# timmh/biolith

Hardware: AMD Instinct MI355X
Metric: effective samples/sec (psi) for occu NUTS, 10k sites x 5 visits (higher is better)
Workload: dtype f32; 1 GPU; biolith simulate(n_sites=10000, n_site_covs=3, n_obs_covs=3, 5 visits, seed 0); fit(occu): NUTS 4 chains per GPU x (1000 warmup + 1000 draws), one step = one full fit; chains_per_gpu=4, total_chains=4, num_warmup=1000, num_samples=1000, parallelism=chains x1 (1 process per GPU), wgs_per_chain=27, gather=none (one rank), env_overrides=

## Files before the change

biolith_amd/_ffi.py:

```python
from __future__ import annotations

import ctypes as C
import os
import threading

_HERE = os.path.dirname(os.path.abspath(__file__))
LIB_PATH = os.environ.get("BIOLITH_HIP_LIB") or os.path.join(_HERE, "lib", "libbiolith_hip.so")

BL_OK, BL_ERR_INVALID, BL_ERR_NO_DEVICE, BL_ERR_UNSUPPORTED, BL_ERR_TIMEOUT, BL_ERR_ABORTED, BL_ERR_BUSY, BL_ERR_COMM = range(8)
COMM_ID_BYTES = 128
RNG_STREAMS_PER_CHAIN = 64
MAX_COVS = 16
PSIS_MAX_DRAWS = 8192
SUMMARY_MAX_RANKS = 16
RICHNESS_MAX_SPECIES = 32


class EngineError(RuntimeError):

    def __init__(self, code: int, message: str):
        super().__init__(f"biolith_hip error {code}: {message}")
        self.code = code


# ... 35 lines not shown
        ("inv_mass", C.POINTER(C.c_float)), ("n_leapfrog", C.POINTER(C.c_int64)),
    ]


EXPORTS = (
    "bl_abi_version", "bl_last_error", "bl_device_count", "bl_dataset_create", "bl_dataset_create_rn", "bl_dataset_create_dyn", "bl_dataset_destroy",
    "bl_dataset_param_dim", "bl_logp_grad", "bl_nuts_run", "bl_nuts_launch", "bl_nuts_poll",
    "bl_nuts_abort", "bl_nuts_wait", "bl_nuts_fetch", "bl_nuts_elapsed_ms", "bl_nuts_device_draws",
    "bl_nuts_geometry", "bl_nuts_lane_group", "bl_nuts_kernel_name", "bl_nuts_debug_counters", "bl_deterministic", "bl_predict", "bl_predict_counts", "bl_predict_scores", "bl_dataset_create_fp", "bl_dataset_create_cop", "bl_dataset_create_nmix", "bl_dataset_create_re", "bl_dataset_create_re_fp", "bl_dataset_create_nmix_re", "bl_dataset_create_rn_re", "bl_dataset_create_rn_fp", "bl_dataset_create_cop_re", "bl_dataset_create_cs", "bl_dataset_create_comb", "bl_dataset_set_prior_family", "bl_rng_streams", "bl_adaptation_schedule",
    "bl_comm_rccl_version", "bl_comm_unique_id", "bl_comm_init_rank", "bl_comm_init_all", "bl_comm_info", "bl_comm_destroy",
    "bl_gather_draws", "bl_result_block_layout", "bl_gather_unpack", "bl_host_alloc", "bl_host_free",
    "bl_nuts_env_overrides", "bl_env_overrides", "bl_site_posterior", "bl_abundance_posterior", "bl_path_posterior",
    "bl_score_posterior", "bl_count_posterior", "bl_predict_comb", "bl_deterministic_comb", "bl_predictive_check",
    "bl_predictive_density", "bl_psis_loo", "bl_predictive_check_counts", "bl_site_summary", "bl_regional_totals",
    "bl_site_diagnostics", "bl_response_curves", "bl_trajectory_totals", "bl_species_richness",
    "bl_residual_moran",
)

_lib = None
_lock = threading.Lock()


def load():
    global _lib
    with _lock:
        if _lib is not None:
            return _lib
        if not os.path.exists(LIB_PATH):
            raise RuntimeError(
                f"{LIB_PATH} is missing: build the HIP engine with `make -C biolith_amd/csrc -j8` "
                "(or `python -c 'import __graft_entry__ as g; g.build()'`). "
# ... 39 lines not shown
        L.bl_logp_grad.argtypes = [vp, C.c_int, dp, dp, dp, C.c_int]
        L.bl_nuts_run.argtypes = [vp, C.POINTER(bl_nuts_config), C.POINTER(bl_nuts_output)]
        L.bl_nuts_launch.argtypes = [vp, C.POINTER(bl_nuts_config), vp]
        L.bl_nuts_poll.argtypes = [vp, ip]
        L.bl_nuts_abort.argtypes = [vp]
        L.bl_nuts_wait.argtypes = [vp]
        L.bl_nuts_fetch.argtypes = [vp, C.POINTER(bl_nuts_output)]
        L.bl_nuts_elapsed_ms.argtypes = [vp, fp]
        L.bl_nuts_device_draws.argtypes = [vp, C.POINTER(vp), C.POINTER(C.c_size_t)]
        L.bl_nuts_geometry.argtypes = [vp, ip, ip, ip, ip, ip]
        L.bl_nuts_lane_group.argtypes = [vp, ip, ip]
        L.bl_nuts_kernel_name.argtypes = [vp, C.c_char_p, C.c_int]
        if hasattr(L, "bl_nuts_env_overrides"):
            L.bl_nuts_env_overrides.argtypes = [vp, C.c_char_p, C.c_int]
            L.bl_env_overrides.argtypes = [C.c_char_p, C.c_int]
        L.bl_nuts_debug_counters.argtypes = [vp, C.POINTER(C.c_int64), C.c_int]
        L.bl_host_alloc.argtypes = [C.c_size_t, C.POINTER(C.c_void_p)]
        L.bl_host_free.argtypes = [C.c_void_p]
        L.bl_deterministic.argtypes = [vp, C.c_int, fp, fp, fp]
        L.bl_predict.argtypes = [vp, C.c_int, fp, C.c_uint64, C.POINTER(C.c_uint8), C.POINTER(C.c_uint8)]
        L.bl_predict_counts.argtypes = [vp, C.c_int, fp, C.c_uint64, C.POINTER(C.c_int32), C.POINTER(C.c_int32)]
        L.bl_predict_scores.argtypes = [vp, C.c_int, fp, C.c_uint64, C.POINTER(C.c_uint8), C.POINTER(C.c_uint8), fp]
        L.bl_predict_comb.argtypes = [vp, C.c_int, fp, C.c_uint64, C.POINTER(C.c_uint8), C.POINTER(C.c_uint8), C.POINTER(C.c_uint8), fp]
        L.bl_deterministic_comb.argtypes = [vp, C.c_int, fp, fp, fp, fp]
        L.bl_predictive_check.argtypes = [vp, C.c_int, fp, C.c_uint64, C.POINTER(C.c_uint8), dp, dp]
        L.bl_predictive_check_counts.argtypes = [vp, C.c_int, fp, C.c_uint64, C.POINTER(C.c_int32), dp, dp]
        L.bl_predictive_density.argtypes = [vp, C.c_int, fp, C.c_uint64, C.POINTER(C.c_uint8), C.c_int, dp, dp, dp]
        L.bl_site_summary.argtypes = [vp, C.c_int, fp, C.c_int, C.POINTER(C.c_int32), dp, dp, fp, dp, dp, fp]
        L.bl_site_diagnostics.argtypes = [vp, C.c_int, fp, C.c_int, dp, dp, dp, dp, dp, dp, dp, dp]
        L.bl_regional_totals.argtypes = [vp, C.c_int, fp, C.c_uint64, C.c_int, C.POINTER(C.c_int32), dp, dp, dp]
# ... 9 lines not shown
        L.bl_score_posterior.argtypes = [vp, C.c_int, fp, C.c_uint64, fp, fp, C.POINTER(C.c_uint8), fp, C.POINTER(C.c_uint8)]
        L.bl_count_posterior.argtypes = [vp, C.c_int, fp, C.c_uint64, fp, fp, C.POINTER(C.c_uint8), fp, C.POINTER(C.c_int32)]
        L.bl_rng_streams.argtypes = [C.c_uint64, C.c_int, C.c_int, C.POINTER(C.c_uint32)]
        L.bl_adaptation_schedule.argtypes = [C.c_int, C.POINTER(C.c_int32), C.POINTER(C.c_int32), C.c_int]
        u8p = C.POINTER(C.c_uint8)
        L.bl_comm_rccl_version.argtypes = [ip]
        L.bl_comm_unique_id.argtypes = [u8p]
        L.bl_comm_init_rank.argtypes = [u8p, C.c_int, C.c_int, C.c_int, C.POINTER(vp)]
        L.bl_comm_init_all.argtypes = [C.c_int, ip, C.POINTER(vp)]
        L.bl_comm_info.argtypes = [vp, ip, ip, ip, dp]
        L.bl_comm_destroy.argtypes = [vp]
        L.bl_gather_draws.argtypes = [C.POINTER(vp), C.POINTER(vp), C.c_int, C.POINTER(C.c_int32), C.POINTER(bl_nuts_output)]
        L.bl_result_block_layout.argtypes = [C.c_int, C.c_int, C.c_int, C.POINTER(C.c_uint64)]
        L.bl_gather_unpack.argtypes = [C.c_void_p, C.c_uint64, C.c_int, C.POINTER(C.c_int32), C.c_int, C.c_int, C.POINTER(bl_nuts_output)]
        for name in EXPORTS:
            if name != "bl_last_error" and (hasattr(L, name) or name not in ("bl_nuts_env_overrides", "bl_env_overrides")):
                getattr(L, name).restype = C.c_int
        if L.bl_abi_version() != 1:
            raise RuntimeError("libbiolith_hip.so ABI version mismatch")
        _lib = L
        return _lib


def check(rc: int):
    if rc != BL_OK:
        msg = load().bl_last_error().decode("utf-8", "replace")
        if rc == BL_ERR_INVALID:
            raise ValueError(f"biolith_hip: {msg}")
        if rc == BL_ERR_UNSUPPORTED:
            raise NotImplementedError(f"biolith_hip: {msg}")
        if rc in (BL_ERR_TIMEOUT,):
# ... 9 lines not shown
```

biolith_amd/csrc/biolith_hip.hip:

```cpp
#include "../../include/biolith_hip.h"

#include <hip/hip_runtime.h>

#include <algorithm>
#include <climits>
#include <cmath>
#include <cstdarg>
#include <cstdio>
#include <cstdlib>
#include <cstring>
#include <string>
#include <vector>

#include "logp_kernel.hpp"
#include "re_kernel.hpp"
#include "nuts_kernel.hpp"
#include "predict.hpp"
#include "site_posterior.hpp"
#include "abundance_posterior.hpp"
#include "path_posterior.hpp"
#include "score_posterior.hpp"
#include "count_posterior.hpp"
#include "comb_predict.hpp"
#include "predictive_check.hpp"
// ... 1895 lines not shown
                 o_cold = carve(sizeof(BlNutsCold));
    if (off > ds->run_bytes) {
        if (ds->d_run) hipFree(ds->d_run);
        ds->d_run = nullptr; ds->run_bytes = 0;
        BL_HIP(hipMalloc(&ds->d_run, off));
        ds->run_bytes = off;
    }
    char *base = (char *)ds->d_run;
    ds->d_draws = (float *)(base + o_draws); ds->d_div = (unsigned char *)(base + o_div); ds->d_steps = (int *)(base + o_steps);
    ds->d_acc = (float *)(base + o_acc); ds->d_pot = (float *)(base + o_pot); ds->d_eps = (float *)(base + o_eps);
    ds->d_minv = (float *)(base + o_minv); ds->d_nleap = (long long *)(base + o_nleap); ds->d_status = (int *)(base + o_status);
    ds->d_rng = (uint32_t *)(base + o_rng); ds->d_init = (float *)(base + o_init); ds->d_dbg = (long long *)(base + o_dbg); ds->d_loc = (int *)(base + o_loc);
    int pitch = nvp;
    { const char *e = bl_env(BL_ENV_PITCH); if (e && atoi(e) >= nvp && atoi(e) <= 4096) pitch = atoi(e); }
    pitch += pitch & 1;
    const size_t xb = align256((size_t)C * BL_XCHG_SLOTS * k * pitch * 8);
    if (xb > ds->xchg_bytes) {
        if (ds->d_xchg) hipFree(ds->d_xchg);
        ds->d_xchg = nullptr; ds->xchg_bytes = 0;
        BL_HIP(hipMalloc((void **)&ds->d_xchg, xb));
        ds->xchg_bytes = xb;
    }

    hipStream_t st = (hipStream_t)stream;
    std::vector<uint32_t> rs((size_t)C * BL_RNG_STREAMS_PER_CHAIN * 4);
    for (int c = 0; c < C; c++)
        rng_streams(cfg->seed, cfg->chain_offset + c, BL_RNG_STREAMS_PER_CHAIN, rs.data() + (size_t)c * BL_RNG_STREAMS_PER_CHAIN * 4);
    BL_HIP(hipMemcpyAsync(ds->d_rng, rs.data(), rs.size() * 4, hipMemcpyHostToDevice, st));
    if (cfg->init_theta) {
        std::vector<float> it32((size_t)C * D);
        for (size_t i = 0; i < it32.size(); i++) it32[i] = (float)cfg->init_theta[i];
// ... 218 lines not shown
{
    if (!ds) return bl_fail(BL_ERR_INVALID, "NULL argument");
    if (!ds->have_run) return bl_fail(BL_ERR_INVALID, "no NUTS launch on this handle");
    if (wgs_per_chain) *wgs_per_chain = ds->k;
    if (threads_per_wg) *threads_per_wg = ds->model == 6 ? BL_RE_NT : 64 * (ds->ncw + 1);
    if (lds_bytes) *lds_bytes = ds->lds_bytes;
    if (lds_staged) *lds_staged = ds->staged;
    if (chains_on_l2_local_exchange) {
        *chains_on_l2_local_exchange = 0;
        if (!ds->in_flight && ds->d_loc) {
            std::vector<int> loc(ds->C, 0);
            BL_HIP(hipMemcpy(loc.data(), ds->d_loc, (size_t)ds->C * 4, hipMemcpyDeviceToHost));
            for (int v : loc) *chains_on_l2_local_exchange += v;
        }
    }
    return BL_OK;
}

extern "C" int bl_deterministic(bl_dataset *ds, int n_draws, const float *draws, float *psi, float *prob_detection)
{
    if (!ds || !draws || n_draws <= 0) return bl_fail(BL_ERR_INVALID, "bl_deterministic: bad argument");
    if (ds->nsp > 1) return bl_fail(BL_ERR_UNSUPPORTED, "bl_deterministic: a joint-species handle samples; take the sites from one handle per species");
    if (ds->model == 8) return bl_fail(BL_ERR_UNSUPPORTED, "bl_deterministic: the dynamic occupancy model's sites (psi, gamma, eps) are formed by the caller from the draws");
    if (ds->model == 6 && ds->re.kind == 8)
        return bl_fail(BL_ERR_UNSUPPORTED, "bl_deterministic: occu_comb's sites (psi, PC / ARU detection probabilities) are formed by the caller from the draws");
    if (ds->in_flight) return bl_fail(BL_ERR_BUSY, "a NUTS launch is in flight on this handle");
    int rc = set_device(ds);
    if (rc || (prob_detection && (rc = upload_once(&ds->d_wraw, ds->h_wraw)))) return rc;
    BlPredictParams p = predict_params(ds, 0);
    const size_t cells = (size_t)p.T * p.N * 4;
// ... 394 lines not shown
```

biolith_amd/csrc/nuts_kernel.hpp:

```cpp
#pragma once
#include "occu_device.hpp"

#ifdef BL_STAMPS
#define BL_STAMP_DECL long long st_acc[8] = {0, 0, 0, 0, 0, 0, 0, 0}; long long st_prev = (long long)clock64(); long long st_rt0 = (long long)wall_clock64(); long long st_spins = 0; \
    long long st_kn[3] = {0, 0, 0}, st_kc[3] = {0, 0, 0}; int st_kind = 0; long long st_sub[6] = {0, 0, 0, 0, 0, 0}; long long st_t = 0; \
    long long st_ae[8] = {0, 0, 0, 0, 0, 0, 0, 0}; int st_ae_cls = -1; \
    long long st_pr[4] = {0, 0, 0, 0}; long long st_bo = 0, st_r0 = 0; bool st_first = true;
#define BL_STAMP_ROUND0 st_r0 = (long long)clock64();
#define BL_STAMP_ROUND1 { const long long st_now = (long long)clock64(); st_sub[3] += st_now - st_r0; \
    if (st_first) { st_pr[0] += st_now - st_r0; st_pr[1] += st_now - st_bo; st_pr[3]++; st_first = false; } else st_pr[2] += st_now - st_r0; }
#define BL_STAMP(i) { const long long st_now = (long long)clock64(); st_acc[i] += st_now - st_prev; \
    if (st_ae_cls >= 0 && (i) <= 1) { st_ae[st_ae_cls * 4 + 1 + ((i) & 1)] += st_now - st_prev; if ((i) == 0) st_ae[st_ae_cls * 4]++; } \
    if ((i) == 5) st_ae_cls = -1; \
    if ((i) == 1) { st_bo = st_now; st_first = true; } \
    st_prev = st_now; }
#define BL_STAMP_AFTER_END(ek) st_ae_cls = ((ek) & 16) ? 1 : (((ek) & 2) ? 0 : -1);
#define BL_STAMP_KIND(k) st_kind = (k);
#define BL_STAMP_CRIT { const long long st_now = (long long)clock64(); st_kn[st_kind]++; st_kc[st_kind] += st_now - st_prev; }
#define BL_COUNT_SPINS(n) { st_spins += (long long)(n); if (st_ae_cls >= 0) st_ae[st_ae_cls * 4 + 3] += (long long)(n); }
#define BL_SUB0 st_t = (long long)clock64();
#define BL_SUB(i) { const long long st_n2 = (long long)clock64(); st_sub[i] += st_n2 - st_t; st_t = st_n2; }
#else
#define BL_SUB0
#define BL_SUB(i)
// ... 143 lines not shown
#define BL_RESIDENT_REC 1
#endif
#ifndef BL_RESIDENT_MAX_FLOATS
#define BL_RESIDENT_MAX_FLOATS 96
#endif
#define SMALL_D_NVP(LEAN, MODEL, KS, KO) ((LEAN) && ((MODEL) == 0 || (MODEL) == 1) && (KS) + (KO) + 2 <= 8)
#ifndef BL_POLL_PAIRS
#define BL_POLL_PAIRS 1
#endif
#ifndef BL_POLL_EARLY
#define BL_POLL_EARLY 0
#endif
#ifndef BL_POLL_REFILL
#define BL_POLL_REFILL 1
#endif
__host__ __device__ __forceinline__ constexpr int bl_pair_pos(int v) { return v < 8 ? 2 * v : 2 * (v - 8) + 1; }
__host__ __device__ __forceinline__ constexpr int bl_pair_lane(int v) { return v < 8 ? v : 24 + v; }
typedef unsigned BlU4 __attribute__((ext_vector_type(4)));
#ifndef BL_OUT_DIRECT
#define BL_OUT_DIRECT 1
#endif
#ifndef BL_ABORT_DEFER
#define BL_ABORT_DEFER 0
#endif
#define BL_ABORT_LAG 8u
typedef __attribute__((address_space(1))) unsigned BlGlobalU;
typedef __attribute__((address_space(1))) unsigned char BlGlobalB;
typedef __attribute__((address_space(1))) const int BlGlobalCI;
#ifndef BL_GRP_FORM
#define BL_GRP_FORM 2
// ... 71 lines not shown
    float pend_dE = 0.f, pend_z = 0.f, pend_g = 0.f;
    double pend_U = 0.0;
    int pend_snprop = 0;
    bool init_pending = true;
    float mom_r0 = 0.f;
    double mom_kin = 0.0;
    int end_kind = 0;
    bool local = false;
    float prior_loc = 0.f, prior_isc2 = 0.f, prior_l1 = 0.f;
    double prior_const = 0.0;
    int S = 0, W = 0, total = 0, nwin = 0, win_end_cur = 0;
    float target_accept = 0.8f;

    const int nvp = SMALL_D_NVP(LEAN, MODEL, KS, KO) ? 16 : p.nvp, G = 64 / nvp;
    const int c_idx = lane & (nvp - 1), sub = lane / nvp;
    const unsigned rec_bytes = (unsigned)(p.k * p.pitch * 8);
    const unsigned char *xbase = reinterpret_cast<const unsigned char *>(p.xchg) + (size_t)chain * BL_XCHG_SLOTS * rec_bytes;
    unsigned poff[8];
    float pval[8];
#pragma unroll
    for (int q = 0; q < 8; q++) {
        const int w = q * G + sub;
        poff[q] = (unsigned)(((w < p.k ? w : p.k - 1) * p.pitch + c_idx) * 8);
        pval[q] = (w < p.k) ? 1.0f : 0.0f;
    }
    const int nq = (p.k + G - 1) / G;
    const bool one_batch = LEAN || p.k <= 8 * G;
    constexpr bool PAIRS = BL_POLL_PAIRS && SMALL_D_NVP(LEAN, MODEL, KS, KO) && multi_wg;
    unsigned ppoff[4] = {0u, 0u, 0u, 0u};
#define BL_XL(v) (PAIRS ? bl_pair_lane(v) : (v))
    if constexpr (PAIRS) {
        const int psub = (lane >> 3) & 3;
#pragma unroll
        for (int q = 0; q < 4; q++) {
            const int w = 4 * (2 * q + (lane >> 5)) + psub;
            ppoff[q] = (unsigned)(((w < p.k ? w : p.k - 1) * p.pitch + 2 * (lane & 7)) * 8);
        }
#pragma unroll
        for (int q = 0; q < 8; q++) pval[q] = (4 * q + psub < p.k) ? 1.0f : 0.0f;
    }

    if (wave == 0) {
        S = cold->num_samples; W = cold->num_warmup; total = W + S;
        target_accept = cold->target_accept; nwin = cold->nwin; win_end_cur = cold->win_end[0];
        prior_loc = beta_lane ? cold->loc_b : cold->loc_a;
        prior_isc2 = act ? (beta_lane ? cold->isc2_b : cold->isc2_a) : 0.0f;
// ... 127 lines not shown
        }
        if (pend_end) {
            const float wt = t_wt;
            float pr = fminf(1.0f, bl_exp(swt - wt));
            if (pend_sturn || pend_sdiv) pr = 0.0f;
            const float u = bl_rng_uniform(rng_u);
            if (u < pr) { t_zp = szp; t_gp = sgp; t_Up = sUp; }
            t_wt = bl_logaddexp(wt, swt);
            t_sumacc += ssumacc;
            t_nprop += pend_snprop;
        }
    };

    unsigned epoch = 0;
    bool have_pending = false, p_timed_out = false;
    double p_acc = 0.0;
    float p_cg = 0.f, p_pe2 = 0.f;
    float cz_spec = 0.f;
    int flag = 0;
    BL_STAMP_DECL
    constexpr bool SPEC = LDS && MODEL != 1;
#ifndef BL_RN_HYBRID
#define BL_RN_HYBRID 2
#endif
    constexpr bool HYBRID = BL_RN_HYBRID && LDS && MODEL == 1;
    constexpr bool POLL_FORMS = SPEC && multi_wg && KS <= 4 && KO <= 4 && MODEL != 8;
    constexpr bool POLL_EARLY = BL_POLL_EARLY && POLL_FORMS;
    constexpr bool POLL_REFILL = BL_POLL_REFILL && POLL_FORMS;
    auto poll_issue_pairs = [&](BlU4 (&v)[4], unsigned ep) {
        const int nqp = (nq + 1) >> 1;
        const __amdgpu_buffer_rsrc_t rsrc = __builtin_amdgcn_make_buffer_rsrc(const_cast<unsigned char *>(xbase), (short)0, (int)(BL_XCHG_SLOTS * rec_bytes), 0x00020000);
        const int soff = __builtin_amdgcn_readfirstlane((int)((ep & (BL_XCHG_SLOTS - 1u)) * rec_bytes));
        asm volatile("" ::: "memory");
#pragma unroll
        for (int q = 0; q < 4; q++) {
            if (q < nqp) v[q] = __builtin_amdgcn_raw_buffer_load_b128(rsrc, (int)ppoff[q], soff, 16);
            else v[q] = BlU4{0u, ep, 0u, ep};
        }
    };
    auto poll_issue_one = [&](unsigned long long (&v)[8], unsigned ep) {
        const unsigned char *rb = xbase + (ep & (BL_XCHG_SLOTS - 1u)) * rec_bytes;
#pragma unroll
        for (int q = 0; q < 8; q += 2) {
            if (q < nq) {
                v[q] = bl_poll_load(rb, poff[q]);
                v[q + 1] = bl_poll_load(rb, poff[q + 1]);
            } else {
                v[q] = (unsigned long long)ep << 32;
                v[q + 1] = (unsigned long long)ep << 32;
            }
        }
    };
    auto poll_fill_one = [&](unsigned long long (&v)[8]) {
#pragma unroll
        for (int q = 2; q < 8; q += 2)
            if (!(q < nq)) { v[q] = v[0]; v[q + 1] = v[0]; }
    };
    auto decide = [&]() {
        have_pending = false;
        const double acc = p_acc;
        const float cg = p_cg, pe2 = p_pe2;
        const double ll_tot = bl_readlane_d(acc, BL_XL(D));
        const bool abort_req = bl_readlane_d(acc, BL_XL(D + 1)) != 0.0;
        flag = 0;
        if (p_timed_out) flag = 4;
        else if (abort_req) flag = 5;
        bool new_transition = false;
        BL_STAMP_KIND(0)
        if (flag == 0) {
            if (init_pending) {
                BL_STAMP_KIND(2)
                BL_SUB0
                const double Un = -ll_tot + (double)(0.5f * bl_wave_sum(pe2)) + prior_const;
                init_pending = false;
                new_transition = true;
                t_zp = cz; t_gp = cg; t_Up = Un;
                end_kind = 1;
            } else {
// ... 100 lines not shown
                epsdir = going_right ? eps : -eps;
                snprop = 0; sturn = false; sdiv = false;
                bl_next_leaf(th, r0, gr, epsdir, minv, rh, cz);
                BL_SUB(2)
            }
        }
        if (flag != 0) end_deferred();
        if (flag != 0 && member == 0) {
            if (flag > 1 && lane == 0) atomicMax(cold->status, flag);
            if (act) cold->inv_mass[chain * D + lane] = minv;
            if (lane == 0) {
                cold->step_size[chain] = eps;
                cold->nleap[chain * 2 + 0] = ss->nleap_w;
                cold->nleap[chain * 2 + 1] = ss->nleap_s;
                cold->xcd_local[chain] = local ? 1 : 0;
            }
        }
    };

    if (wave > 0) {
        if constexpr (BL_COMPUTE_PRIO > 0 && MODEL != 1 && multi_wg) __builtin_amdgcn_s_setprio(BL_COMPUTE_PRIO);
        unsigned epoch_c = 0;
        const int lane_grp = MODEL == 1 ? bl_rn_npos(p.rn_off) : p.lane_grp;
        BlPairRec<KS, KO, (RESIDENT ? JSEL : 1)> rrec;
        bool rvalid = false;
        float rvmask = 0.0f;
        if constexpr (RESIDENT) bl_load_resident_rec(tid - 64, ld, cnt, rrec, rvalid, rvmask);
        int ab_raw = 0;
        const unsigned ab_mask = (__builtin_amdgcn_readfirstlane(wave) == 1 && member == 0) ? 0u : 0x80000000u;
        while (true) {
// ... 19 lines not shown
            if (lane == 0) tags[wave - 1] = epoch_c;
            unsigned stale = 0u;
#pragma unroll
            for (int w = 0; w < CW; w++) stale |= tags[w] ^ epoch_c;
            float row[CW];
#pragma unroll
            for (int w = 0; w < CW; w++) row[w] = part[w * part_rs];
            if (__builtin_amdgcn_readfirstlane(stale) == 0u) {
                float comp = row[0];
#pragma unroll
                for (int w = 1; w < CW; w++) comp += row[w];
                for (int sp = 1; sp < nsp; sp++) {
#pragma unroll
                    for (int w = 0; w < CW; w++) comp += part_all ? (float)part[w * part_rs + sp * BL_SP_PART(KS, KO)] : 0.0f;
                }
                if (lane > D) comp = 0.0f;
                if constexpr (ABORT_DEFER) {
                    if (lane == D + 1 && member == 0 && (epoch_c & 255u) == BL_ABORT_LAG + 1u)
                        comp = (*(__attribute__((address_space(3))) const volatile int *)(sh_flag + 2) != 0) ? 1.0f : 0.0f;
                } else {
                    if (lane == D + 1 && member == 0 && (epoch_c & 255u) == 0u)
                        comp = (__hip_atomic_load(cold->abort_flag, __ATOMIC_RELAXED, __HIP_MEMORY_SCOPE_SYSTEM) != 0) ? 1.0f : 0.0f;
                }
                if (epoch_c == 1u) {
                    const float xcc = (float)bl_xcc_id();
                    if (lane == D + 2) comp = xcc;
                    if (lane == D + 3) comp = xcc * xcc;
                }
                const unsigned char *rbase = xbase + (epoch_c & (BL_XCHG_SLOTS - 1u)) * rec_bytes;
                const unsigned long long granule = ((unsigned long long)epoch_c << 32) | __float_as_uint(comp);
                if (lane < nvp) {
                    int lane_o = lane;
                    asm volatile("" : "+v"(lane_o));
                    const int gran = lane_o & (nvp - 1);
                    const unsigned store_off = (unsigned)((member * p.pitch + (PAIRS ? bl_pair_pos(gran) : gran)) * 8);
                    unsigned long long *dst = reinterpret_cast<unsigned long long *>(const_cast<unsigned char *>(rbase) + store_off);
                    if (local_c)
                        __hip_atomic_store(dst, granule, __ATOMIC_RELAXED, __HIP_MEMORY_SCOPE_WORKGROUP);
                    else
                        __hip_atomic_store(dst, granule, __ATOMIC_RELAXED, __HIP_MEMORY_SCOPE_AGENT);
                }
            }
            }
            __syncthreads();
            if constexpr (ABORT_DEFER) {
                const unsigned ph = (epoch_c & 255u) | ab_mask;
                if (__builtin_expect(ph <= BL_ABORT_LAG, 0)) {
                    if (ph == 0u) {
                        const unsigned *abw = reinterpret_cast<const unsigned *>(bl_lds_f(BL_OFF_SV)) + SV_ABORT * 64;
                        BlGlobalCI *ab_ptr = (BlGlobalCI *)(((size_t)abw[1] << 32) | abw[0]);
                        if (lane == 0) ab_raw = __hip_atomic_load(ab_ptr, __ATOMIC_RELAXED, __HIP_MEMORY_SCOPE_SYSTEM);
                    } else if (ph == BL_ABORT_LAG) {
                        if (lane == 0 && ab_raw != 0) sh_flag[2] = 1;
                    }
                }
// ... 21 lines not shown
            BL_STAMP_AFTER_END(end_kind)
            end_deferred();
            BL_STAMP(0)
        }
        float pe2 = 0.0f, pg = 0.0f;
        int spec_kind = 0;
        float spec_ed = epsdir, spec_other = 0.0f;
        BlU4 pv[4];
        unsigned long long ov[8];
        const bool early = POLL_EARLY && (PAIRS || one_batch) && (BL_POLL_EARLY != 2 || (decided && snprop == 0));
        if (!redo) {
        if constexpr (POLL_EARLY) {
            if (early) {
                for (int z = 0; z < p.first_delay; z++) __builtin_amdgcn_s_sleep(1);
                BL_STAMP_ROUND0
                if (PAIRS) poll_issue_pairs(pv, epoch + 1u);
                else poll_issue_one(ov, epoch + 1u);
                BL_STAMP(6)
            }
        }
        const float dth = cz - prior_loc;
        pe2 = fmaf(dth * dth, prior_isc2, 2.0f * fabsf(dth) * prior_l1);
        pg = fmaf(dth, prior_isc2, dth > 0.0f ? prior_l1 : (dth < 0.0f ? -prior_l1 : 0.0f));
        if constexpr (MODEL == 2) {
            if (is_phi) {
                const float e = bl_exp(-fabsf(cz)), op = 1.0f + e, l = bl_log(op);
                const float sig = (cz > 0.0f ? 1.0f : e) * bl_rcp(op);
                pe2 = 2.0f * (prior_loc * (fmaxf(-cz, 0.0f) + l) + prior_isc2 * (fmaxf(cz, 0.0f) + l));
                pg = (prior_loc + prior_isc2) * sig - prior_loc;
            }
        }
// ... 27 lines not shown
        }
        __syncthreads();
        BL_STAMP(1)

        epoch++;
        if (redo) {
            if (act) sh_coef[my_pos] = cz;
            if (lane == 0) sh_flag[0] = flag;
            run_status = flag;
        } else {
            const unsigned char *rbase = xbase + (epoch & (BL_XCHG_SLOTS - 1u)) * rec_bytes;
            BL_STAMP(2)
            if (!early)
                for (int z = 0; z < p.first_delay; z++) __builtin_amdgcn_s_sleep(1);
            double acc = 0.0;
            bool timed_out = false;
            if (!multi_wg) {
                const float *part = bl_lds_f(BL_OFF_PART) + part_pos;
                float comp = part[0];
#pragma unroll
                for (int w = 1; w < CW; w++) comp += part[w * part_rs];
                for (int sp = 1; sp < nsp; sp++) {
#pragma unroll
                    for (int w = 0; w < CW; w++) comp += part_all ? part[w * part_rs + sp * BL_SP_PART(KS, KO)] : 0.0f;
                }
                if (lane > D) comp = 0.0f;
                if constexpr (ABORT_DEFER) {
                    if (lane == D + 1 && (epoch & 255u) == BL_ABORT_LAG + 1u)
                        comp = (*(__attribute__((address_space(3))) const volatile int *)(sh_flag + 2) != 0) ? 1.0f : 0.0f;
                } else {
                    if (lane == D + 1 && (epoch & 255u) == 0u)
                        comp = (__hip_atomic_load(cold->abort_flag, __ATOMIC_RELAXED, __HIP_MEMORY_SCOPE_SYSTEM) != 0) ? 1.0f : 0.0f;
                }
                acc = (double)comp;
            } else if (PAIRS && (POLL_EARLY || POLL_REFILL)) {
                const __amdgpu_buffer_rsrc_t rsrc = __builtin_amdgcn_make_buffer_rsrc(const_cast<unsigned char *>(xbase), (short)0, (int)(BL_XCHG_SLOTS * rec_bytes), 0x00020000);
                const int soff = __builtin_amdgcn_readfirstlane((int)((epoch & (BL_XCHG_SLOTS - 1u)) * rec_bytes));
                BlSpinBound bound;
                if (!early) {
                    BL_STAMP_ROUND0
                    poll_issue_pairs(pv, epoch);
                }
                while (true) {
                    unsigned badq[4], bad = 0u;
#pragma unroll
                    for (int q = 0; q < 4; q++) {
                        badq[q] = (pv[q].y ^ epoch) | (pv[q].w ^ epoch);
                        bad |= badq[q];
                    }
// ... 148 lines not shown
                        for (int q = 0; q < 8; q++) {
                            const int w = p0 + (b * 8 + q) * G + sub;
                            acc += (w < p.k) ? (double)__uint_as_float((unsigned)v[b][q]) : 0.0;
                        }
                }
            }
            if (PAIRS) {
                acc += bl_dpp_d<0x128, 0xF>(acc);
                acc = bl_fold_rows16_d(acc);
            } else if (multi_wg) {
                if (nvp <= 16) acc = bl_fold_rows16_d(acc);
                if (nvp <= 32) acc = bl_fold_halves32_d(acc);
            }
            BL_STAMP(3)
            if (epoch == 1u && p.allow_local) {
                const double sx = bl_readlane_d(acc, BL_XL(D + 2)), sxx = bl_readlane_d(acc, BL_XL(D + 3));
                local = ((double)p.k * sxx == sx * sx);
                if (lane == 0) sh_flag[1] = local ? 1 : 0;
            }
            const float cg = act ? (-(float)acc + pg) : 0.0f;
            p_acc = acc; p_cg = cg; p_pe2 = pe2; p_timed_out = timed_out;
            have_pending = true;
            cz_spec = __builtin_nanf("");
            if (!SPEC && !(HYBRID && spec_kind != 0 && !timed_out)) {
                decide();
                if (act) sh_coef[my_pos] = cz;
                if (lane == 0) sh_flag[0] = flag;
                run_status = flag;
                BL_STAMP_CRIT
            } else {
            if (spec_kind != 0 && !timed_out) {
// ... 49 lines not shown
```

biolith_amd/engine.py:

```python
from __future__ import annotations

import ctypes as C
import time
from dataclasses import dataclass
from typing import Optional, Sequence

import numpy as np

from . import _ffi


def _fp(a):
    return a.ctypes.data_as(C.POINTER(C.c_float)) if a is not None else None


def _dp(a):
    return a.ctypes.data_as(C.POINTER(C.c_double)) if a is not None else None


class _PinnedPool:

    def __init__(self, cap=1 << 30):
        import threading

# ... 58 lines not shown
    potential_energy: np.ndarray
    step_size: np.ndarray
    inv_mass: np.ndarray
    n_leapfrog: np.ndarray
    kernel_ms: float
    wgs_per_chain: int
    lds_bytes: int
    lds_staged: bool
    chains_l2_local: int = 0
    threads_per_wg: int = 0
    lds_vector_tier: int = 0
    comm_init_ms: float = 0.0
    lane_group: tuple = (1, 1)
    kernel_name: str = ""
    env_overrides: str = ""


class OccuDataset:

    def __init__(self, site_covs, obs_covs, obs, prior_beta=(0.0, 1.0), prior_alpha=(0.0, 1.0), device: int = 0,
                 model: str = "occu", max_abundance: int = 100, fp_mode: Optional[str] = "constant", prior_fp=(2.0, 5.0),
                 session_duration=None, prior_fp_rate: float = 1.0, site_random_effects: bool = False,
                 obs_random_effects: bool = False, prior_site_re_sd: float = 1.0, prior_obs_re_sd: float = 1.0,
                 prior_mu=((0.0, 10.0), (0.0, 10.0)), prior_sigma=((5.0, 1.0), (5.0, 1.0)), re_fp_mode: Optional[str] = None,
                 ARU_obs_covs=None, ARU_obs=None, scores_obs=None, prior_fc=(2.0, 5.0), prior_fu=(2.0, 5.0)):
        lib = _ffi.load()
        if model not in ("occu", "occu_rn", "occu_fp", "occu_cop", "nmixture", "occu_re", "occu_cs", "occu_dyn", "occu_comb"):
            raise ValueError(f"unknown model {model!r}")
        if fp_mode not in ("constant", "unoccupied") and not (model == "occu_cop" and fp_mode is None):
            raise ValueError(f"unknown fp_mode {fp_mode!r}")
# ... 207 lines not shown
        _ffi.check(self._lib.bl_nuts_geometry(self._h, C.byref(k), C.byref(thr), C.byref(lds), C.byref(staged), C.byref(loc)))
        return int(k.value)

    def _kernel_name(self) -> str:
        buf = C.create_string_buffer(192)
        _ffi.check(self._lib.bl_nuts_kernel_name(self._h, buf, 192))
        return buf.value.decode()

    def env_overrides(self) -> str:
        if not hasattr(self._lib, "bl_nuts_env_overrides"):
            return ""
        buf = C.create_string_buffer(512)
        _ffi.check(self._lib.bl_nuts_env_overrides(self._h, buf, 512))
        return buf.value.decode()

    def elapsed_ms(self) -> float:
        ms = C.c_float(0)
        _ffi.check(self._lib.bl_nuts_elapsed_ms(self._h, C.byref(ms)))
        return float(ms.value)

    def debug_counters(self, n: int = 32):
        out = np.zeros(n, dtype=np.int64)
        _ffi.check(self._lib.bl_nuts_debug_counters(self._h, out.ctypes.data_as(C.POINTER(C.c_int64)), n))
        return out

    def device_draws(self):
        p, n = C.c_void_p(), C.c_size_t()
        _ffi.check(self._lib.bl_nuts_device_draws(self._h, C.byref(p), C.byref(n)))
        return p.value, n.value

# ... 6 lines not shown
        out = _ffi.bl_nuts_output(
            _fp(a["draws"]), a["diverging"].ctypes.data_as(C.POINTER(C.c_uint8)), a["num_steps"].ctypes.data_as(C.POINTER(C.c_int32)),
            _fp(a["accept_prob"]), _fp(a["potential_energy"]), _fp(a["step_size"]), _fp(a["inv_mass"]),
            a["n_leapfrog"].ctypes.data_as(C.POINTER(C.c_int64)),
        )
        return a, out

    def _result(self, a) -> NutsResult:
        k, thr, lds, staged, loc = C.c_int(), C.c_int(), C.c_int(), C.c_int(), C.c_int()
        _ffi.check(self._lib.bl_nuts_geometry(self._h, C.byref(k), C.byref(thr), C.byref(lds), C.byref(staged), C.byref(loc)))
        gt, gj = C.c_int(1), C.c_int(1)
        _ffi.check(self._lib.bl_nuts_lane_group(self._h, C.byref(gt), C.byref(gj)))
        return NutsResult(a["draws"], a["diverging"].astype(bool), a["num_steps"], a["accept_prob"], a["potential_energy"],
                          a["step_size"], a["inv_mass"], a["n_leapfrog"], self.elapsed_ms(),
                          k.value, lds.value, bool(staged.value & 1), loc.value, thr.value, staged.value >> 1,
                          lane_group=(int(gt.value), int(gj.value)), kernel_name=self._kernel_name(), env_overrides=self.env_overrides())

    def fetch(self) -> NutsResult:
        Cn, S = self._shape
        a, out = self._output(Cn, S)
        _ffi.check(self._lib.bl_nuts_fetch(self._h, C.byref(out)))
        return self._result(a)

    def nuts(self, timeout: Optional[float] = None, **kw) -> NutsResult:
        self.launch(**kw)
        if timeout is not None:
            t_end = time.monotonic() + float(timeout)
            try:
                while not self.done():
                    if time.monotonic() > t_end:
                        raise TimeoutError("Timed out")
# ... 320 lines not shown
```

include/biolith_hip.h:

```cpp
#ifndef BIOLITH_HIP_H
#define BIOLITH_HIP_H

#include <stddef.h>
#include <stdint.h>

#ifdef __cplusplus
extern "C" {
#endif

#define BL_ABI_VERSION 1

enum {
    BL_OK = 0,
    BL_ERR_INVALID = 1,
    BL_ERR_NO_DEVICE = 2,
    BL_ERR_UNSUPPORTED = 3,
    BL_ERR_TIMEOUT = 4,
    BL_ERR_ABORTED = 5,
    BL_ERR_BUSY = 6,
    BL_ERR_COMM = 7
};

#define BL_RNG_STREAMS_PER_CHAIN 64
#define BL_MAX_COVS 16
// ... 107 lines not shown
    float *inv_mass;
    int64_t *n_leapfrog;
} bl_nuts_output;

int bl_nuts_run(bl_dataset *ds, const bl_nuts_config *cfg, bl_nuts_output *out);

int bl_nuts_launch(bl_dataset *ds, const bl_nuts_config *cfg, void *stream);
int bl_nuts_poll(bl_dataset *ds, int *done);
int bl_nuts_abort(bl_dataset *ds);
int bl_nuts_wait(bl_dataset *ds);
int bl_nuts_fetch(bl_dataset *ds, bl_nuts_output *out);
int bl_nuts_elapsed_ms(bl_dataset *ds, float *ms);
int bl_nuts_device_draws(bl_dataset *ds, void **dev_ptr, size_t *bytes);
int bl_nuts_geometry(bl_dataset *ds, int *wgs_per_chain, int *threads_per_wg, int *lds_bytes, int *lds_staged,
                     int *chains_on_l2_local_exchange);

int bl_nuts_lane_group(bl_dataset *ds, int *period_lanes, int *visit_lanes);

int bl_nuts_kernel_name(bl_dataset *ds, char *buf, int n);

int bl_nuts_env_overrides(bl_dataset *ds, char *buf, int n);
int bl_env_overrides(char *buf, int n);

int bl_host_alloc(size_t bytes, void **out);
int bl_host_free(void *ptr);

int bl_nuts_debug_counters(bl_dataset *ds, int64_t *out , int n);

int bl_deterministic(bl_dataset *ds, int n_draws, const float *draws, float *psi, float *prob_detection);

// ... 86 lines not shown
```

Measured before the change: 293,200 ESS/s.

## Pack cross-workgroup exchange records into compact 2 KB slots for occupancy model

Adds a compact exchange format for the multi-workgroup pairs path of the occupancy model. Each workgroup's partial sums, log-likelihood bits, abort flag and XCC id are packed into eight 16-byte granules per member, with epoch tags, inside a fixed 2 KB slot. The poller then reads two 128-bit buffer loads per lane instead of the pitched per-parameter layout, and unpacks with DPP and permlane32 swaps. This is meant to shrink exchange traffic and polling latency per leapfrog step. The cost is more complex packing, with the log-likelihood split into 16-bit halves. A new record_bytes query reports the record size.

After: 299,700 ESS/s (median of 6 runs). 2.2% higher.

```diff
diff --git a/biolith_amd/_ffi.py b/biolith_amd/_ffi.py
--- a/biolith_amd/_ffi.py
+++ b/biolith_amd/_ffi.py
@@ -73,7 +73,7 @@
     "bl_score_posterior", "bl_count_posterior", "bl_predict_comb", "bl_deterministic_comb", "bl_predictive_check",
     "bl_predictive_density", "bl_psis_loo", "bl_predictive_check_counts", "bl_site_summary", "bl_regional_totals",
     "bl_site_diagnostics", "bl_response_curves", "bl_trajectory_totals", "bl_species_richness",
-    "bl_residual_moran",
+    "bl_residual_moran", "bl_nuts_record_bytes",
 )
 
 _lib = None
@@ -143,6 +143,8 @@
         if hasattr(L, "bl_nuts_env_overrides"):
             L.bl_nuts_env_overrides.argtypes = [vp, C.c_char_p, C.c_int]
             L.bl_env_overrides.argtypes = [C.c_char_p, C.c_int]
+        if hasattr(L, "bl_nuts_record_bytes"):
+            L.bl_nuts_record_bytes.argtypes = [vp, ip]
         L.bl_nuts_debug_counters.argtypes = [vp, C.POINTER(C.c_int64), C.c_int]
         L.bl_host_alloc.argtypes = [C.c_size_t, C.POINTER(C.c_void_p)]
         L.bl_host_free.argtypes = [C.c_void_p]
@@ -182,7 +184,7 @@
         L.bl_result_block_layout.argtypes = [C.c_int, C.c_int, C.c_int, C.POINTER(C.c_uint64)]
         L.bl_gather_unpack.argtypes = [C.c_void_p, C.c_uint64, C.c_int, C.POINTER(C.c_int32), C.c_int, C.c_int, C.POINTER(bl_nuts_output)]
         for name in EXPORTS:
-            if name != "bl_last_error" and (hasattr(L, name) or name not in ("bl_nuts_env_overrides", "bl_env_overrides")):
+            if name != "bl_last_error" and (hasattr(L, name) or name not in ("bl_nuts_env_overrides", "bl_env_overrides", "bl_nuts_record_bytes")):
                 getattr(L, name).restype = C.c_int
         if L.bl_abi_version() != 1:
             raise RuntimeError("libbiolith_hip.so ABI version mismatch")
diff --git a/biolith_amd/csrc/biolith_hip.hip b/biolith_amd/csrc/biolith_hip.hip
--- a/biolith_amd/csrc/biolith_hip.hip
+++ b/biolith_amd/csrc/biolith_hip.hip
@@ -1933,7 +1933,8 @@
     int pitch = nvp;
     { const char *e = bl_env(BL_ENV_PITCH); if (e && atoi(e) >= nvp && atoi(e) <= 4096) pitch = atoi(e); }
     pitch += pitch & 1;
-    const size_t xb = align256((size_t)C * BL_XCHG_SLOTS * k * pitch * 8);
+    const size_t xb_pitched = (size_t)C * BL_XCHG_SLOTS * k * pitch * 8, xb_compact = (size_t)C * BL_XCHG_SLOTS * BL_COMPACT_SLOT_BYTES;
+    const size_t xb = align256(xb_pitched > xb_compact ? xb_pitched : xb_compact);
     if (xb > ds->xchg_bytes) {
         if (ds->d_xchg) hipFree(ds->d_xchg);
         ds->d_xchg = nullptr; ds->xchg_bytes = 0;
@@ -2182,6 +2183,18 @@
             for (int v : loc) *chains_on_l2_local_exchange += v;
         }
     }
+    return BL_OK;
+}
+
+extern "C" int bl_nuts_record_bytes(bl_dataset *ds, int *record_bytes)
+{
+    if (!ds || !record_bytes) return bl_fail(BL_ERR_INVALID, "NULL argument");
+    if (!ds->have_run || ds->in_flight) return bl_fail(BL_ERR_BUSY, "no finished NUTS launch");
+    int rc = set_device(ds);
+    if (rc) return rc;
+    int said = 0;
+    if (ds->model != 6) BL_HIP(hipMemcpy(&said, ds->d_status + 1, 4, hipMemcpyDeviceToHost));
+    *record_bytes = said > 0 ? said : ds->nvp * 8;
     return BL_OK;
 }
 
diff --git a/biolith_amd/csrc/nuts_kernel.hpp b/biolith_amd/csrc/nuts_kernel.hpp
--- a/biolith_amd/csrc/nuts_kernel.hpp
+++ b/biolith_amd/csrc/nuts_kernel.hpp
@@ -181,6 +181,14 @@
 #ifndef BL_POLL_REFILL
 #define BL_POLL_REFILL 1
 #endif
+#ifndef BL_POLL_COMPACT
+#define BL_POLL_COMPACT 1
+#endif
+#define BL_COMPACT_SLOT_BYTES 2048u
+__host__ __device__ __forceinline__ constexpr unsigned bl_compact_off(int w, int d)
+{
+    return 16u * (unsigned)((((w & 3) * 4 + (w >> 3)) * 8) + d) + 8u * (unsigned)((w >> 2) & 1);
+}
 __host__ __device__ __forceinline__ constexpr int bl_pair_pos(int v) { return v < 8 ? 2 * v : 2 * (v - 8) + 1; }
 __host__ __device__ __forceinline__ constexpr int bl_pair_lane(int v) { return v < 8 ? v : 24 + v; }
 typedef unsigned BlU4 __attribute__((ext_vector_type(4)));
@@ -282,7 +290,9 @@
 
     const int nvp = SMALL_D_NVP(LEAN, MODEL, KS, KO) ? 16 : p.nvp, G = 64 / nvp;
     const int c_idx = lane & (nvp - 1), sub = lane / nvp;
-    const unsigned rec_bytes = (unsigned)(p.k * p.pitch * 8);
+    constexpr bool PAIRS = BL_POLL_PAIRS && SMALL_D_NVP(LEAN, MODEL, KS, KO) && multi_wg;
+    constexpr bool COMPACT = BL_POLL_COMPACT && PAIRS && MODEL == 0;
+    const unsigned rec_bytes = COMPACT ? BL_COMPACT_SLOT_BYTES : (unsigned)(p.k * p.pitch * 8);
     const unsigned char *xbase = reinterpret_cast<const unsigned char *>(p.xchg) + (size_t)chain * BL_XCHG_SLOTS * rec_bytes;
     unsigned poff[8];
     float pval[8];
@@ -294,10 +304,19 @@
     }
     const int nq = (p.k + G - 1) / G;
     const bool one_batch = LEAN || p.k <= 8 * G;
-    constexpr bool PAIRS = BL_POLL_PAIRS && SMALL_D_NVP(LEAN, MODEL, KS, KO) && multi_wg;
     unsigned ppoff[4] = {0u, 0u, 0u, 0u};
-#define BL_XL(v) (PAIRS ? bl_pair_lane(v) : (v))
-    if constexpr (PAIRS) {
+    unsigned cmask[2] = {0u, 0u};
+#define BL_XL(v) (COMPACT ? 33 : PAIRS ? bl_pair_lane(v) : (v))
+    if constexpr (COMPACT) {
+        const int psub = (lane >> 3) & 3, ph = lane >> 5;
+#pragma unroll
+        for (int j = 0; j < 2; j++) {
+            ppoff[j] = bl_compact_off(4 * (2 * (2 * ph + j)) + psub, lane & 7);
+            cmask[j] = ((4 * (2 * (2 * ph + j)) + psub < p.k) ? 0xFFFFu : 0u) | ((4 * (2 * (2 * ph + j) + 1) + psub < p.k) ? 0xFFFF0000u : 0u);
+        }
+#pragma unroll
+        for (int q = 0; q < 8; q++) pval[q] = (4 * q + psub < p.k) ? 1.0f : 0.0f;
+    } else if constexpr (PAIRS) {
         const int psub = (lane >> 3) & 3;
 #pragma unroll
         for (int q = 0; q < 4; q++) {
@@ -455,6 +474,7 @@
 
     unsigned epoch = 0;
     bool have_pending = false, p_timed_out = false;
+    bool p_abort = false;
     double p_acc = 0.0;
     float p_cg = 0.f, p_pe2 = 0.f;
     float cz_spec = 0.f;
@@ -479,6 +499,14 @@
             else v[q] = BlU4{0u, ep, 0u, ep};
         }
     };
+    auto poll_issue_compact = [&](BlU4 (&v)[4], unsigned ep) {
+        const __amdgpu_buffer_rsrc_t rsrc = __builtin_amdgcn_make_buffer_rsrc(const_cast<unsigned char *>(xbase), (short)0, (int)(BL_XCHG_SLOTS * BL_COMPACT_SLOT_BYTES), 0x00020000);
+        const int soff = __builtin_amdgcn_readfirstlane((int)((ep & (BL_XCHG_SLOTS - 1u)) * BL_COMPACT_SLOT_BYTES));
+        asm volatile("" ::: "memory");
+        v[0] = __builtin_amdgcn_raw_buffer_load_b128(rsrc, (int)ppoff[0], soff, 16);
+        if (p.k > 8) v[1] = __builtin_amdgcn_raw_buffer_load_b128(rsrc, (int)ppoff[1], soff, 16);
+        else v[1] = BlU4{0u, 0u, 0u, 0u};
+    };
     auto poll_issue_one = [&](unsigned long long (&v)[8], unsigned ep) {
         const unsigned char *rb = xbase + (ep & (BL_XCHG_SLOTS - 1u)) * rec_bytes;
 #pragma unroll
@@ -502,7 +530,7 @@
         const double acc = p_acc;
         const float cg = p_cg, pe2 = p_pe2;
         const double ll_tot = bl_readlane_d(acc, BL_XL(D));
-        const bool abort_req = bl_readlane_d(acc, BL_XL(D + 1)) != 0.0;
+        const bool abort_req = COMPACT ? p_abort : (bl_readlane_d(acc, BL_XL(D + 1)) != 0.0);
         flag = 0;
         if (p_timed_out) flag = 4;
         else if (abort_req) flag = 5;
@@ -633,6 +661,7 @@
                 cold->nleap[chain * 2 + 0] = ss->nleap_w;
                 cold->nleap[chain * 2 + 1] = ss->nleap_s;
                 cold->xcd_local[chain] = local ? 1 : 0;
+                if constexpr (COMPACT) cold->status[1] = 64;
             }
         }
     };
@@ -682,6 +711,36 @@
 #pragma unroll
                     for (int w = 0; w < CW; w++) comp += part_all ? (float)part[w * part_rs + sp * BL_SP_PART(KS, KO)] : 0.0f;
                 }
+                if constexpr (COMPACT) {
+                    const unsigned llb = (unsigned)__builtin_amdgcn_readlane((int)__float_as_uint(comp), D);
+                    unsigned pay = lane == 0 ? llb << 16 : (lane == 1 ? (llb & 0xFFFF0000u) : 0u);
+                    if (lane >= D) comp = 0.0f;
+                    if constexpr (ABORT_DEFER) {
+                        if (lane == 2 && member == 0 && (epoch_c & 255u) == BL_ABORT_LAG + 1u)
+                            pay = (*(__attribute__((address_space(3))) const volatile int *)(sh_flag + 2) != 0) ? 0x10000u : 0u;
+                    } else {
+                        if (member == 0 && (epoch_c & 255u) == 0u) {
+                            const unsigned abw = (unsigned)__builtin_amdgcn_readfirstlane(__hip_atomic_load(cold->abort_flag, __ATOMIC_RELAXED, __HIP_MEMORY_SCOPE_SYSTEM));
+                            if (lane == 2) pay = abw != 0u ? 0x10000u : 0u;
+                        }
+                    }
+                    if (epoch_c == 1u) {
+                        const unsigned xcc = bl_xcc_id();
+                        if (lane == 3) pay = xcc << 16;
+                        if (lane == 4) pay = (xcc * xcc) << 16;
+                    }
+                    const unsigned hi = pay | (epoch_c & 0xFFFFu);
+                    const unsigned char *rbase = xbase + (epoch_c & (BL_XCHG_SLOTS - 1u)) * BL_COMPACT_SLOT_BYTES;
+                    const unsigned long long granule = ((unsigned long long)hi << 32) | __float_as_uint(comp);
+                    if (lane < 8) {
+                        int lane_o = lane;
+                        asm volatile("" : "+v"(lane_o));
+                        const unsigned store_off = bl_compact_off(member, 0) + 16u * (unsigned)(lane_o & 7);
+                        unsigned long long *dst = reinterpret_cast<unsigned long long *>(const_cast<unsigned char *>(rbase) + store_off);
+                        if (local_c) __hip_atomic_store(dst, granule, __ATOMIC_RELAXED, __HIP_MEMORY_SCOPE_WORKGROUP);
+                        else __hip_atomic_store(dst, granule, __ATOMIC_RELAXED, __HIP_MEMORY_SCOPE_AGENT);
+                    }
+                } else {
                 if (lane > D) comp = 0.0f;
                 if constexpr (ABORT_DEFER) {
                     if (lane == D + 1 && member == 0 && (epoch_c & 255u) == BL_ABORT_LAG + 1u)
@@ -707,6 +766,7 @@
                         __hip_atomic_store(dst, granule, __ATOMIC_RELAXED, __HIP_MEMORY_SCOPE_WORKGROUP);
                     else
                         __hip_atomic_store(dst, granule, __ATOMIC_RELAXED, __HIP_MEMORY_SCOPE_AGENT);
+                }
                 }
             }
             }
@@ -758,7 +818,8 @@
             if (early) {
                 for (int z = 0; z < p.first_delay; z++) __builtin_amdgcn_s_sleep(1);
                 BL_STAMP_ROUND0
-                if (PAIRS) poll_issue_pairs(pv, epoch + 1u);
+                if (COMPACT) poll_issue_compact(pv, epoch + 1u);
+                else if (PAIRS) poll_issue_pairs(pv, epoch + 1u);
                 else poll_issue_one(ov, epoch + 1u);
                 BL_STAMP(6)
             }
@@ -816,6 +877,7 @@
             if (!early)
                 for (int z = 0; z < p.first_delay; z++) __builtin_amdgcn_s_sleep(1);
             double acc = 0.0;
+            double cen_sx = 0.0, cen_sxx = 0.0;
             bool timed_out = false;
             if (!multi_wg) {
                 const float *part = bl_lds_f(BL_OFF_PART) + part_pos;
@@ -835,6 +897,62 @@
                         comp = (__hip_atomic_load(cold->abort_flag, __ATOMIC_RELAXED, __HIP_MEMORY_SCOPE_SYSTEM) != 0) ? 1.0f : 0.0f;
                 }
                 acc = (double)comp;
+            } else if (COMPACT) {
+                const __amdgpu_buffer_rsrc_t rsrc = __builtin_amdgcn_make_buffer_rsrc(const_cast<unsigned char *>(xbase), (short)0, (int)(BL_XCHG_SLOTS * BL_COMPACT_SLOT_BYTES), 0x00020000);
+                const int soff = __builtin_amdgcn_readfirstlane((int)((epoch & (BL_XCHG_SLOTS - 1u)) * BL_COMPACT_SLOT_BYTES));
+                BlSpinBound bound;
+                if (!early) {
+                    BL_STAMP_ROUND0
+                    poll_issue_compact(pv, epoch);
+                }
+                while (true) {
+                    const unsigned ep2 = (epoch & 0xFFFFu) * 0x10001u;
+                    unsigned badq[2];
+#pragma unroll
+                    for (int j = 0; j < 2; j++) badq[j] = (__builtin_amdgcn_perm(pv[j].w, pv[j].y, 0x05040100u) ^ ep2) & cmask[j];
+                    const bool all_in = __all((badq[0] | badq[1]) == 0u);
+                    BL_STAMP_ROUND1
+                    if (all_in) break;
+                    if (bound.expired(p.spin_limit)) { timed_out = true; break; }
+                    if (!local)
+                        for (int z = 0; z < p.poll_sleep; z++) __builtin_amdgcn_s_sleep(1);
+                    BL_STAMP_ROUND0
+                    if constexpr (POLL_REFILL) {
+                        asm volatile("" ::: "memory");
+#pragma unroll
+                        for (int j = 0; j < 2; j++) {
+                            if (badq[j] != 0u) pv[j] = __builtin_amdgcn_raw_buffer_load_b128(rsrc, (int)ppoff[j], soff, 16);
+                        }
+                    } else {
+                        poll_issue_compact(pv, epoch);
+                    }
+                }
+                BL_COUNT_SPINS(bound.spins)
+                p_abort = ((unsigned)__builtin_amdgcn_readlane((int)pv[0].y, 2) >> 16) != 0u;
+                if (epoch == 1u && p.allow_local) {
+                    float xs = 0.0f;
+#pragma unroll
+                    for (int j = 0; j < 2; j++)
+                        xs += ((cmask[j] & 0xFFFFu) ? (float)(pv[j].y >> 16) : 0.0f) + ((cmask[j] >> 16) ? (float)(pv[j].w >> 16) : 0.0f);
+                    cen_sx = (double)bl_wave_sum((lane & 7) == 3 ? xs : 0.0f);
+                    cen_sxx = (double)bl_wave_sum((lane & 7) == 4 ? xs : 0.0f);
+                }
+                unsigned cval[4], cll[4];
+#pragma unroll
+                for (int i = 0; i < 4; i++) {
+                    const unsigned hi = (i & 1) ? pv[i >> 1].w : pv[i >> 1].y;
+                    cval[i] = (i & 1) ? pv[i >> 1].z : pv[i >> 1].x;
+                    cll[i] = (hi & 0xFFFF0000u) | ((unsigned)__builtin_amdgcn_update_dpp(0, (int)hi, 0x111, 0xF, 0xF, false) >> 16);
+                }
+                unsigned cup[4];
+#pragma unroll
+                for (int i = 0; i < 4; i++) {
+                    const auto r = __builtin_amdgcn_permlane32_swap(cval[i], cll[i], false, false);
+                    acc += (double)(pval[i] * __uint_as_float(r[0]));
+                    cup[i] = r[1];
+                }
+#pragma unroll
+                for (int i = 0; i < 4; i++) acc += (double)(pval[4 + i] * __uint_as_float(cup[i]));
             } else if (PAIRS && (POLL_EARLY || POLL_REFILL)) {
                 const __amdgpu_buffer_rsrc_t rsrc = __builtin_amdgcn_make_buffer_rsrc(const_cast<unsigned char *>(xbase), (short)0, (int)(BL_XCHG_SLOTS * rec_bytes), 0x00020000);
                 const int soff = __builtin_amdgcn_readfirstlane((int)((epoch & (BL_XCHG_SLOTS - 1u)) * rec_bytes));
@@ -1013,7 +1131,7 @@
             }
             BL_STAMP(3)
             if (epoch == 1u && p.allow_local) {
-                const double sx = bl_readlane_d(acc, BL_XL(D + 2)), sxx = bl_readlane_d(acc, BL_XL(D + 3));
+                const double sx = COMPACT ? cen_sx : bl_readlane_d(acc, BL_XL(D + 2)), sxx = COMPACT ? cen_sxx : bl_readlane_d(acc, BL_XL(D + 3));
                 local = ((double)p.k * sxx == sx * sx);
                 if (lane == 0) sh_flag[1] = local ? 1 : 0;
             }
diff --git a/biolith_amd/engine.py b/biolith_amd/engine.py
--- a/biolith_amd/engine.py
+++ b/biolith_amd/engine.py
@@ -96,6 +96,7 @@
     lane_group: tuple = (1, 1)
     kernel_name: str = ""
     env_overrides: str = ""
+    record_bytes: int = 0
 
 
 class OccuDataset:
@@ -333,6 +334,13 @@
         _ffi.check(self._lib.bl_nuts_env_overrides(self._h, buf, 512))
         return buf.value.decode()
 
+    def record_bytes(self) -> int:
+        if not hasattr(self._lib, "bl_nuts_record_bytes"):
+            return 0
+        n = C.c_int(0)
+        _ffi.check(self._lib.bl_nuts_record_bytes(self._h, C.byref(n)))
+        return int(n.value)
+
     def elapsed_ms(self) -> float:
         ms = C.c_float(0)
         _ffi.check(self._lib.bl_nuts_elapsed_ms(self._h, C.byref(ms)))
@@ -369,7 +377,8 @@
         return NutsResult(a["draws"], a["diverging"].astype(bool), a["num_steps"], a["accept_prob"], a["potential_energy"],
                           a["step_size"], a["inv_mass"], a["n_leapfrog"], self.elapsed_ms(),
                           k.value, lds.value, bool(staged.value & 1), loc.value, thr.value, staged.value >> 1,
-                          lane_group=(int(gt.value), int(gj.value)), kernel_name=self._kernel_name(), env_overrides=self.env_overrides())
+                          lane_group=(int(gt.value), int(gj.value)), kernel_name=self._kernel_name(), env_overrides=self.env_overrides(),
+                          record_bytes=self.record_bytes())
 
     def fetch(self) -> NutsResult:
         Cn, S = self._shape
diff --git a/include/biolith_hip.h b/include/biolith_hip.h
--- a/include/biolith_hip.h
+++ b/include/biolith_hip.h
@@ -145,6 +145,7 @@
 int bl_nuts_device_draws(bl_dataset *ds, void **dev_ptr, size_t *bytes);
 int bl_nuts_geometry(bl_dataset *ds, int *wgs_per_chain, int *threads_per_wg, int *lds_bytes, int *lds_staged,
                      int *chains_on_l2_local_exchange);
+int bl_nuts_record_bytes(bl_dataset *ds, int *record_bytes);
 
 int bl_nuts_lane_group(bl_dataset *ds, int *period_lanes, int *visit_lanes);
 
```
